# 0xPolygonZero/proof-protocol-decoder

Measured on AMD Instinct MI355X. Metric: txn-proofs/sec (whole node), 256-txn synthetic block, higher is better.
Workload: dtype u64 (Goldilocks field)

## Files before the change

### include/bpg.h

```cpp
#ifndef BPG_H
#define BPG_H
#include <stddef.h>
#include <stdint.h>

#ifdef __cplusplus
extern "C" {
#endif

typedef enum {
  BP_OK = 0,
  BP_ERR_ABORTED = -1,
  BP_ERR_INVALID_INPUT = -2,
  BP_ERR_RANGE = -3,
  BP_ERR_DEVICE = -4,
  BP_ERR_VERIFY = -5,
  BP_ERR_UNSUPPORTED = -6
} bp_status;

const char* bp_last_error(void);
const char* bp_version(void);
int bp_device_count(void);
int bp_use_blocking_sync(int device);
int bp_host_wait_mode(int device);



#define BP_NTT_MAX_COLS 65535u

enum { BP_NTT_FWD_BR2NAT = 0, BP_NTT_INV_NAT2BR = 1, BP_NTT_FWD_NAT = 2, BP_NTT_INV_NAT = 3 };
int bp_ntt_batch(uint64_t* d_cols, uint32_t log_n, uint32_t n_cols, uint64_t col_stride, int dir,
                 void* stream);

int bp_intt_batch(const uint64_t* d_values, uint64_t in_stride, uint64_t* d_coeffs_out, uint64_t out_stride,
                  uint32_t log_n, uint32_t n_cols, void* stream);

int bp_lde_batch(const uint64_t* d_in, uint64_t in_stride, uint64_t* d_coeffs_out, uint64_t coeffs_stride,
                 uint64_t* d_lde_out, uint64_t lde_stride, uint32_t log_n, uint32_t rate_bits,
                 uint32_t n_cols, int from_coeffs, void* stream);

int bp_debug_copy_u64(const uint64_t* d_in, uint64_t* d_out, uint64_t n, void* stream);

int bp_debug_field_ops(const uint64_t* d_a, const uint64_t* d_b, uint64_t* d_out, uint64_t n, void* stream);
int bp_debug_lazy_forms(const uint64_t* d_a, const uint64_t* d_b, uint64_t* d_out, uint64_t n, void* stream);
int bp_debug_mul_pow2(const uint64_t* d_a, uint64_t* d_out, uint64_t n, void* stream);

void bp_tune_quad_threshold(uint64_t n_perms);
void bp_tune_merkle_fused(int mode);
void bp_tune_merkle_wide(int log2_parents);
void bp_tune_poseidon_mx(int on);
void bp_tune_poseidon_mx_sets(int sets);
void bp_tune_poseidon_grouped(int on);
void bp_tune_assume_loaded(int mode);
void bp_tune_rec_batch(int n);
void bp_tune_side_lanes(int n);
void bp_tune_rec_riders(int on);
void bp_tune_txn_group(int n);
void bp_tune_rec_group(int mode);
int bp_debug_rec_batch_histogram(uint64_t* out, uint32_t n, int reset);
void bp_tune_witness_threads(int n);
void bp_tune_host_wait(int mode);
void bp_tune_host_poseidon(int mode);
int bp_debug_poseidon_host(uint64_t* states, size_t n);
void bp_tune_k5_spread(int on);
uint32_t bp_debug_poseidon_group_ops(uint32_t K);
int bp_debug_poseidon_group_tables(uint32_t K, uint32_t r0, uint8_t* out_ops, int32_t* out_cform, int32_t* out_cmain,
                                   int32_t* out_max_plane_sum);

void bp_tune_ntt_split(int mode);
void bp_tune_ntt_mx(int mode);
void bp_tune_reset(void);
int bp_debug_tune_state(char* buf, size_t cap);
int bp_debug_ntt_mx_tables(int kind, int inverse, uint8_t* out_a, int32_t* out_c, uint64_t* out_tw256,
                           uint64_t* out_tw16);
int bp_debug_poseidon_mx_cin(uint32_t* out);

int bp_poseidon_perm_batch(uint64_t* d_states, uint64_t n, void* stream);

uint64_t bp_merkle_digest_words(uint32_t log_leaves, uint32_t cap_height);
int bp_merkle_commit(const uint64_t* d_lde, uint64_t lde_stride, uint32_t n_cols, uint32_t log_n,
                     uint32_t rate_bits, uint32_t cap_height, uint64_t* d_digests, void* stream);

struct bp_stark_cfg;
typedef struct bp_air_family {
  uint32_t first_index, count;
  uint32_t kind;
  uint32_t degree;
} bp_air_family;
typedef struct bp_air_desc {
  uint32_t air_id;
  char name[24];
  uint32_t fixed_n_cols;
  uint32_t n_const_max;
  uint32_t degree;
  uint32_t n_cols, n_aux;
  uint32_t n_air_constraints, n_ctl_constraints;
  uint32_t n_units;
  uint32_t n_families;
  bp_air_family families[24];
} bp_air_desc;
uint32_t bp_air_count(void);
int bp_air_describe(uint32_t air_id, uint32_t n_cols, uint32_t n_const, uint32_t deg_pow, bp_air_desc* out);

int bp_air_register(const uint64_t* program, size_t n_words, uint32_t* air_id_out);
int bp_air_unregister(uint32_t air_id);
int bp_air_program_digest(uint32_t air_id, uint8_t out[32]);

uint64_t bp_quotient_scratch_words(uint32_t air_id, const struct bp_stark_cfg* shape);
int bp_quotient_eval(uint32_t air_id, const struct bp_stark_cfg* shape, const uint64_t* d_trace_lde,
                     const uint64_t* d_aux_lde, const uint64_t* d_const_lde, const uint64_t ctl[4],
                     const uint64_t alphas[2], uint64_t* d_scratch, uint64_t* d_qvals_out, void* stream);

int bp_air_port_products(uint32_t air_id, const struct bp_stark_cfg* shape, const uint64_t* d_trace, uint64_t stride,
                         const uint64_t* d_consts, const uint64_t pub[4], const uint64_t ctl[4], uint64_t* d_aux_out, void* stream);

int bp_range_multiplicities(const uint64_t* d_values, uint64_t stride, uint32_t n_cols, uint64_t n_rows, const uint64_t* d_filter,
                            uint32_t log_range, uint64_t* d_mult, uint64_t* first_bad, void* stream);
void bp_tune_range_lds_log(int log_range);

int bp_debug_air_aux(uint32_t air_id, const struct bp_stark_cfg* shape, const uint64_t* d_trace, const uint64_t ctl[4],
                     uint64_t* d_aux_out, void* stream);

typedef struct bp_air_violation {
  uint32_t row, constraint, family, kind;
  uint64_t value;
} bp_air_violation;
int bp_air_check_trace(uint32_t air_id, const struct bp_stark_cfg* shape, const uint64_t* d_trace, uint64_t stride,
                       const uint64_t* d_consts, const uint64_t pub[4], uint32_t max_rows, uint64_t* n_violated_rows,
// ... 274 lines not shown
```

### proof_protocol_decoder_amd/_abi.py

```python
import ctypes as C
from ctypes import POINTER as P

vp, cp, i, sz, dbl = C.c_void_p, C.c_char_p, C.c_int, C.c_size_t, C.c_double
u8, u32, u64, i32, i64 = C.c_uint8, C.c_uint32, C.c_uint64, C.c_int32, C.c_int64
u8p, u32p, u64p, i32p, szp = P(u8), P(u32), P(u64), P(i32), P(sz)
u8pp = P(u8p)

BP_OK, BP_ERR_ABORTED, BP_ERR_INVALID_INPUT, BP_ERR_RANGE, BP_ERR_DEVICE, BP_ERR_VERIFY, BP_ERR_UNSUPPORTED = 0, -1, -2, -3, -4, -5, -6
STATUS_NAMES = {v: k for k, v in list(globals().items()) if k == "BP_OK" or k.startswith("BP_ERR_")}
BP_SET_SKIP_LINK_CHECK = 1
BP_NUM_TABLES, BP_IR_WORDS, BP_PV_WORDS = 7, 25, 13

KNOBS = ("quad_threshold", "assume_loaded", "merkle_fused", "merkle_wide", "poseidon_mx", "poseidon_mx_sets",
         "poseidon_grouped", "ntt_mx", "ntt_split", "k5_spread", "host_wait", "host_poseidon", "rec_batch",
         "witness_threads", "side_lanes")


def _u32s(*names):
    return [(n, u32) for n in names]


class AirFamily(C.Structure):
    _fields_ = _u32s("first_index", "count", "kind", "degree")

# ... 94 lines not shown
    _fields_ = [("txn_number", u64), ("gas_used", u64), ("state_root", u64 * 4)]


class ShardOptions(C.Structure):
    _fields_ = _u32s("n_threads", "tree_shape")


ShardLeafFn = C.CFUNCTYPE(i, vp, u32, u8pp, szp)
ShardAggFn = C.CFUNCTYPE(i, vp, u8p, sz, i, u8p, sz, i, u8pp, szp)

_cfg, _conf, _wit, _opt, _gi = P(StarkCfg), P(BpConfig), P(TxnWitness), P(ShardOptions), P(GiOptions)
_trace = (i, [vp, u64, u32, vp, vp])
_check = [u32, _cfg, vp, u64, vp, u64p, u32, u64p, u32p, P(AirViolation), u32, u32p]
_knob, _ir_flag, _buf = (None, [i]), (i, [u64p, i]), [u8pp, szp]
PROTOTYPES = {
    "bp_last_error": (cp, []),
    "bp_version": (cp, []),
    "bp_device_count": (i, []),
    "bp_use_blocking_sync": (i, [i]),
    "bp_host_wait_mode": (i, [i]),
    "bp_ntt_batch": (i, [vp, u32, u32, u64, i, vp]),
    "bp_intt_batch": (i, [vp, u64, vp, u64, u32, u32, vp]),
    "bp_lde_batch": (i, [vp, u64, vp, u64, vp, u64, u32, u32, u32, i, vp]),
    "bp_debug_copy_u64": (i, [vp, vp, u64, vp]),
    "bp_debug_field_ops": (i, [vp, vp, vp, u64, vp]),
    "bp_debug_lazy_forms": (i, [vp, vp, vp, u64, vp]),
    "bp_debug_mul_pow2": (i, [vp, vp, u64, vp]),
    "bp_tune_quad_threshold": (None, [u64]),
    "bp_tune_merkle_fused": _knob,
    "bp_tune_merkle_wide": _knob,
    "bp_tune_poseidon_mx": _knob,
    "bp_tune_poseidon_mx_sets": _knob,
    "bp_tune_poseidon_grouped": _knob,
    "bp_tune_assume_loaded": _knob,
    "bp_tune_rec_batch": _knob,
    "bp_tune_side_lanes": _knob,
    "bp_tune_rec_riders": _knob,
    "bp_tune_txn_group": _knob,
    "bp_tune_rec_group": _knob,
    "bp_debug_rec_batch_histogram": (i, [u64p, u32, i]),
    "bp_tune_witness_threads": _knob,
    "bp_tune_host_wait": _knob,
    "bp_tune_host_poseidon": _knob,
    "bp_debug_poseidon_host": (i, [vp, sz]),
    "bp_tune_k5_spread": _knob,
    "bp_debug_poseidon_group_ops": (u32, [u32]),
    "bp_debug_poseidon_group_tables": (i, [u32, u32, u8p, i32p, i32p, i32p]),
    "bp_tune_ntt_split": _knob,
    "bp_tune_ntt_mx": _knob,
    "bp_tune_reset": (None, []),
    "bp_debug_tune_state": (i, [cp, sz]),
    "bp_debug_ntt_mx_tables": (i, [i, i, u8p, i32p, u64p, u64p]),
    "bp_debug_poseidon_mx_cin": (i, [u32p]),
    "bp_poseidon_perm_batch": (i, [vp, u64, vp]),
    "bp_merkle_digest_words": (u64, [u32, u32]),
    "bp_merkle_commit": (i, [vp, u64, u32, u32, u32, u32, vp, vp]),
    "bp_air_count": (u32, []),
    "bp_air_describe": (i, [u32, u32, u32, u32, P(AirDesc)]),
    "bp_air_register": (i, [vp, sz, u32p]),
    "bp_air_unregister": (i, [u32]),
    "bp_air_program_digest": (i, [u32, cp]),
    "bp_quotient_scratch_words": (u64, [u32, _cfg]),
    "bp_quotient_eval": (i, [u32, _cfg, vp, vp, vp, u64p, u64p, vp, vp, vp]),
    "bp_air_port_products": (i, [u32, _cfg, vp, u64, vp, u64p, u64p, vp, vp]),
    "bp_range_multiplicities": (i, [vp, u64, u32, u64, vp, u32, vp, u64p, vp]),
    "bp_tune_range_lds_log": _knob,
    "bp_debug_air_aux": (i, [u32, _cfg, vp, u64p, vp, vp]),
    "bp_air_check_trace": (i, _check + [vp]),
    "bp_air_check_trace_host": (i, _check),
    "bp_keccak_trace": _trace,
    "bp_logic_trace": _trace,
    "bp_memory_trace": _trace,
    "bp_arithmetic_trace": _trace,
    "bp_byte_packing_trace": _trace,
    "bp_keccak_sponge_trace": _trace,
    "bp_arithmetic_mul_trace": _trace,
    "bp_arithmetic_div_trace": (i, [vp, u32, vp, vp]),
    "bp_arithmetic_div_layout": (i, [u32p, sz]),
    "bp_arithmetic_mod_trace": (i, [vp, u32, vp, vp]),
    "bp_arithmetic_mod_layout": (i, [u32p, sz]),
    "bp_arithmetic_shift_trace": (i, [vp, u32, vp, vp]),
    "bp_arithmetic_shift_layout": (i, [u32p, sz]),
    "bp_arithmetic_sdiv_trace": (i, [vp, u32, vp, vp]),
    "bp_arithmetic_sdiv_layout": (i, [u32p, sz]),
    "bp_arithmetic_exp_trace": (i, [vp, u32, vp, u32, vp, vp]),
    "bp_arithmetic_exp_layout": (i, [u32p, sz]),
    "bp_plonk_constants": (i, [u64, u32, P(PlonkLayout), vp, vp]),
    "bp_plonk_trace": (i, [vp, u64, u64p, P(PlonkLayout), u64p, u32, vp, vp]),
    "bp_fri_fold": (i, [vp, u32, u32, u32, u64, u64p, vp, vp]),
    "bp_openings": (i, [vp, u64, u32, u32, u64p, u64p, vp, vp, vp]),
    "bp_pow_grind": (i, [u64p, u32, u32, u64p, vp]),
    "bp_stark_prove_synthetic": (i, [_cfg, u64, u64, i] + _buf),
    "bp_stark_prove_air": (i, [u32, _cfg, u64, u64, i] + _buf),
    "bp_stark_prove_trace": (i, [u32, _cfg, vp, u64, vp, u64p, i] + _buf),
    "bp_stark_verify_air": (i, [u32, _cfg, u64p, cp, sz]),
    "bp_stark_public_inputs": (None, [u64, u64p]),
    "bp_stark_public_input_list": (None, [u64, u64p]),
    "bp_stark_verify_air_pub": (i, [u32, _cfg, u64p, u64p, cp, sz]),
    "bp_stark_prove_table_set": (i, [P(SetTable), u32, P(SetLink), u32, u32, i] + _buf),
    "bp_stark_verify_table_set": (i, [P(SetTable), u32, P(u64p), P(SetLink), u32, cp, sz]),
    "bp_check_table_set": (i, [P(SetTable), u32, P(SetLink), u32, i, P(SetReport)]),
    "bp_release_cached_memory": (None, []),
    "bp_free_buffer": (None, [u8p]),
    "bp_config_default": (None, [_conf]),
    "bp_state_build": (i, [_conf, P(vp)]),
    "bp_state_free": (None, [vp]),
# ... 54 lines not shown
```

### proof_protocol_decoder_amd/csrc/air.hpp

```cpp
#pragma once
#include <cstdint>
#include <type_traits>
#include "gl.hpp"
#if defined(__HIP__)
#include "poseidon.cuh"
#endif

namespace bpg {
namespace air {

constexpr uint32_t SYNTHETIC = 0, KECCAK_F = 1, LOGIC = 2, MEMORY = 3, ARITHMETIC = 4, BYTE_PACKING = 5, KECCAK_SPONGE = 6, ARITHMETIC_MUL = 7, PLONK = 8, COUNT = 9;

struct Shape {
  uint32_t air_id, n_cols, n_const, deg_pow;
};

template <class T>
struct Ops;

#if defined(__HIP__)
template <>
struct Ops<uint64_t> {
  typedef uint64_t T;
  static __device__ __forceinline__ T k(uint64_t c) { return c; }
  static __device__ __forceinline__ T add(T a, T b) { return gl::addc(a, b); }
  static __device__ __forceinline__ T sub(T a, T b) { return gl::subc(a, b); }
  static __device__ __forceinline__ T mul(T a, T b) { return gl::mulc(a, b); }
  static __device__ __forceinline__ T dbl(T a) { return gl::addc(a, a); }
  static __device__ __forceinline__ void mul4(const T (&a)[4], const T (&b)[4], T (&r)[4]) {
    __builtin_amdgcn_sched_barrier(0);
    gl::mul_n<4>(a, b, r);
    gl::canon_n<4>(r);
    __builtin_amdgcn_sched_barrier(0);
  }
  static __device__ __forceinline__ void mul4_lazy(const T (&a)[4], const T (&b)[4], T (&r)[4]) {
    __builtin_amdgcn_sched_barrier(0);
    gl::mul_n<4>(a, b, r);
    __builtin_amdgcn_sched_barrier(0);
  }
  static __device__ __forceinline__ T add_lazy(T a_any, T b) { return gl::add(a_any, b); }
  static __device__ __forceinline__ T sub_lazy(T a_any, T b) { return gl::sub(a_any, b); }
  static __device__ __forceinline__ T mul7(T a_any) { return gl::mul7(a_any); }
};
#endif
template <>
struct Ops<gl::Ext> {
  typedef gl::Ext T;
  static T k(uint64_t c) { return gl::ext(c); }
  static T add(T a, T b) { return gl::add(a, b); }
  static T sub(T a, T b) { return gl::sub(a, b); }
  static T mul(T a, T b) { return gl::mul(a, b); }
  static T dbl(T a) { return gl::add(a, a); }
  static void mul4(const T (&a)[4], const T (&b)[4], T (&r)[4]) {
    for (int i = 0; i < 4; i++) r[i] = gl::mul(a[i], b[i]);
  }
  static void mul4_lazy(const T (&a)[4], const T (&b)[4], T (&r)[4]) { mul4(a, b, r); }
  static T add_lazy(T a, T b) { return gl::add(a, b); }
  static T sub_lazy(T a, T b) { return gl::sub(a, b); }
  static T mul7(T a) { return gl::scale(a, 7); }
};

GL_HD uint64_t poseidon_rc(uint32_t i) {
  constexpr uint64_t RC[360] = {
#include "poseidon_rc.inc"
  };
  return RC[i];
}
GL_HD uint32_t poseidon_mds_entry(uint32_t r, uint32_t c) {
  constexpr uint32_t C[12] = {17, 15, 41, 16, 2, 28, 13, 13, 39, 18, 34, 20};
  return C[(c + 12 - r) % 12] + ((r | c) == 0 ? 8u : 0u);
}
template <class T>
struct PoseidonOps {
  typedef Ops<T> F;
  static GL_HD T sbox(T x) {
    const T x2 = F::mul(x, x), x4 = F::mul(x2, x2), x3 = F::mul(x2, x);
    return F::mul(x3, x4);
  }
  static GL_HD void sbox_all(T (&s)[12]) {
    for (uint32_t i = 0; i < 12; i++) s[i] = sbox(s[i]);
  }
  static GL_HD void mds_rc(T (&s)[12], int next) {
    T o[12];
    for (uint32_t r = 0; r < 12; r++) {
      T acc = F::k(next >= 0 ? poseidon_rc(12 * (uint32_t)next + r) : 0);
      for (uint32_t c = 0; c < 12; c++) acc = F::add(acc, F::mul(F::k(poseidon_mds_entry(r, c)), s[c]));
      o[r] = acc;
    }
    for (uint32_t r = 0; r < 12; r++) s[r] = o[r];
  }
  static GL_HD void mds_rc_word0(T (&s)[12], int next) { mds_rc(s, next); }
  static GL_HD T add_rc0(T x, uint32_t i) { return F::add(x, F::k(poseidon_rc(i))); }
};
#if defined(__HIP__)
template <>
struct PoseidonOps<uint64_t> {
  static __device__ __forceinline__ uint64_t sbox(uint64_t x) { return gl::canon(poseidon::sbox(x)); }
  static __device__ __forceinline__ void sbox_all(uint64_t (&s)[12]) { poseidon::sbox_all(s); }
  static __device__ __forceinline__ void mds_rc(uint64_t (&s)[12], int next) {
    if (next >= 0) poseidon::mds<true>(s, poseidon::RC + 12 * next);
    else poseidon::mds<false>(s, nullptr);
#pragma unroll
    for (int i = 0; i < 12; i++) s[i] = gl::canon(s[i]);
  }
  static __device__ __forceinline__ void mds_rc_word0(uint64_t (&s)[12], int next) {
    poseidon::mds<true>(s, poseidon::RC + 12 * next);
    s[0] = gl::canon(s[0]);
  }
  static __device__ __forceinline__ uint64_t add_rc0(uint64_t x, uint32_t i) { return gl::addc(x, poseidon::RC[i]); }
};
#endif

namespace synthetic {
GL_HD uint32_t n_constraints(const Shape& s) { return 3 * (s.n_cols / 4); }
GL_HD uint32_t per_unit(const Shape& s) {
  const uint32_t G = s.n_cols / 4, u = (G + 47) / 48;
  return u < 8 ? 8 : u;
}
GL_HD uint32_t n_units(const Shape& s) {
  const uint32_t G = s.n_cols / 4, pu = per_unit(s);
  return (G + pu - 1) / pu;
}
template <class T, class Row, class Emit>
GL_HD void eval_unit(const Shape& s, uint32_t unit, const Row& row, Emit& out) {
  typedef Ops<T> F;
  const uint32_t G = s.n_cols / 4, pu = per_unit(s), g0 = unit * pu, g1 = g0 + pu < G ? g0 + pu : G;
#pragma unroll 1
  for (uint32_t g = g0; g < g1; g++) {
    const T a = row.loc(4 * g), b = row.loc(4 * g + 1), c = row.loc(4 * g + 2), d = row.loc(4 * g + 3);
    const T dn = row.nxt(4 * g + 3);
    const T q = s.n_const ? row.cst(g % s.n_const) : F::k(1);
    const T x4[4] = {a, q, a, a}, y4[4] = {b, a, b, b};
    T p4[4];
    F::mul4(x4, y4, p4);
    const T ab = p4[0], qa = p4[1];
    T t = F::mul(ab, c);
    if (s.deg_pow == 3) t = F::mul(F::mul(t, t), t);
    out.all(3 * g, F::sub(F::sub(c, ab), qa));
    out.transition(3 * g + 1, F::sub(F::sub(dn, t), b));
    out.first(3 * g + 2, F::sub(F::sub(d, a), b));
  }
}
}

namespace keccak {
constexpr uint32_t N_COLS = 2431, N_CONSTRAINTS = 2826, N_UNITS = 11;
constexpr uint32_t COL_STEP = 0, COL_A = 24, COL_C = 74, COL_CP = 394, COL_AP = 714, COL_APP = 2314, COL_APP0_BITS = 2364,
                   COL_APPP = 2428, COL_G = 2430;
constexpr uint32_t F0 = 0, F1 = 24, F2 = 48, F3 = 2032, F4 = 2352, F5 = 2672, F6 = 2722, F7 = 2772, F8 = 2774, F9 = 2776;
GL_HD uint64_t round_constant(uint32_t i) {
  constexpr uint64_t RC[24] = {
      0x0000000000000001ULL, 0x0000000000008082ULL, 0x800000000000808aULL, 0x8000000080008000ULL,
      0x000000000000808bULL, 0x0000000080000001ULL, 0x8000000080008081ULL, 0x8000000000008009ULL,
      0x000000000000008aULL, 0x0000000000000088ULL, 0x0000000080008009ULL, 0x000000008000000aULL,
      0x000000008000808bULL, 0x800000000000008bULL, 0x8000000000008089ULL, 0x8000000000008003ULL,
      0x8000000000008002ULL, 0x8000000000000080ULL, 0x000000000000800aULL, 0x800000008000000aULL,
      0x8000000080008081ULL, 0x8000000000008080ULL, 0x0000000080000001ULL, 0x8000000080008008ULL};
  return RC[i];
}
GL_HD uint32_t rho(uint32_t l) {
  constexpr uint8_t R[25] = {0, 1, 62, 28, 27, 36, 44, 6, 55, 20, 3, 10, 43, 25, 39, 41, 45, 15, 21, 8, 18, 2, 61, 56, 14};
  return R[l];
// ... 607 lines not shown
        const uint32_t j = col - H_OUT;
        if (l + 1 == L.depth) { const uint32_t i = L.path_pi0 + 8 * p + 4 + j; col_out = i & 7; row_out = HASH_ROW0 + (i >> 3); }
        else { col_out = H_IN + j; row_out = row + 1; }
      }
    } else if (L.leaf_len && row >= leaf_row0(L) && row < leaf_row0(L) + leaf_rows(L)) {
      const uint32_t LH = hash_rows(L.leaf_len), t = row - leaf_row0(L), p = t / LH, h = t % LH;
      if (col < 12) {
        if (hash_word_is_carried(L.leaf_len, h, col)) {
          if (h > 0) { col_out = H_OUT + col; row_out = row - 1; }
          else if (col < 11) col_out = col + 1;
          else if (p + 1 < L.n_paths) { col_out = 8; row_out = row + LH; }
          else { col_out = MERKLE_ZERO_COL; row_out = ZERO_ROW; }
        }
      } else if (col < 24) {
        const uint32_t k = col - H_OUT;
        if (h + 1 == LH) {
          if (k < 4) { const uint32_t i = L.path_pi0 + 8 * p + k; col_out = i & 7; row_out = HASH_ROW0 + (i >> 3); }
        } else if (hash_word_is_carried(L.leaf_len, h + 1, k)) {
          col_out = H_IN + k; row_out = row + 1;
        }
      }
    }
    return;
  }
  const uint32_t g = row >> 2, p = row & 3, s = col >> 2, w = col & 3;
  const uint32_t base = 4 * g;
  if (p == 0) {
    if (w == 3) { col_out = 4 * s; row_out = base + 1; }
    else if (w == 2) { col_out = col; row_out = base + 1; }
  } else if (p == 1) {
    if (w == 0) { col_out = 4 * ((s + N_SLOTS - 1) % N_SLOTS) + 1; row_out = base + 1; }
    else if (w == 1) { col_out = 4 * ((s + 1) % N_SLOTS) + 3; row_out = base; }
    else if (w == 2) {
      if (base == A0 && s < 4) { col_out = H_OUT + s; row_out = last_hash_row; }
      else { col_out = col; row_out = base; }
    } else if (s < N_SBOX) { col_out = 4 * s; row_out = base + 2; }
  } else if (p == 2) {
    if (s < N_SBOX && w == 0) { col_out = 4 * s + 3; row_out = base + 1; }
    else if (s < N_SBOX && w == 3) { col_out = 4 * s; row_out = base + 3; }
  } else {
    if (s < N_SBOX && w == 0) { col_out = 4 * s + 3; row_out = base + 2; }
  }
}
GL_HD uint64_t chunk_shift(uint32_t u) {
  constexpr uint64_t K8[10] = {0x1ULL, 0x57f6c1ULL, 0x1e39a5057d81ULL, 0x62b942f056949437ULL, 0x33cdc3006affab59ULL,
                               0xcb893e19494e73dULL, 0x36f01f6fb02d9400ULL, 0xd844c68aea81b372ULL, 0x9c232dfb69ab851eULL,
                               0x255bd1d3b936892aULL};
  return K8[u];
}
template <class T, class Row, class Emit, bool SELECTOR = true>
GL_HD void eval_hash_unit(const Row& row, Emit& out) {
  typedef Ops<T> F;
  typedef PoseidonOps<T> H;
  const T qh = row.cst(CST_HASH);
  const T q4[4] = {qh, qh, qh, qh};
  T st[12];
  {
    const T sw = row.loc(H_SWAP);
    T lhs[4], rhs[4], dl[4], pr[4], g[4];
#pragma unroll
    for (uint32_t i = 0; i < 4; i++) {
      lhs[i] = row.loc(H_IN + i);
      rhs[i] = row.loc(H_IN + 4 + i);
      dl[i] = row.loc(H_DELTA + i);
      pr[i] = F::sub(rhs[i], lhs[i]);
    }
    const T s4[4] = {sw, sw, sw, sw};
    F::mul4(s4, pr, g);
#pragma unroll
    for (uint32_t i = 0; i < 4; i++) {
      const T d = F::sub(dl[i], g[i]);
      out.all(G5 + 1 + i, SELECTOR ? F::mul(qh, d) : d);
      st[i] = H::add_rc0(F::add(lhs[i], dl[i]), i);
      st[4 + i] = H::add_rc0(F::sub(rhs[i], dl[i]), 4 + i);
      st[8 + i] = H::add_rc0(row.loc(H_IN + 8 + i), 8 + i);
    }
    const T bit = F::mul(sw, F::sub(sw, F::k(1)));
    out.all(G5, SELECTOR ? F::mul(qh, bit) : bit);
  }
  auto check12 = [&](uint32_t col0, uint32_t idx0) {
#pragma unroll
    for (uint32_t i0 = 0; i0 < 12; i0 += 4) {
      T d[4], g[4];
#pragma unroll
      for (uint32_t i = 0; i < 4; i++) {
        const T wv = row.loc(col0 + i0 + i);
        d[i] = F::sub(wv, st[i0 + i]);
        st[i0 + i] = wv;
      }
      if (SELECTOR) F::mul4(q4, d, g);
#pragma unroll
      for (uint32_t i = 0; i < 4; i++) out.all(idx0 + i0 + i, SELECTOR ? g[i] : d[i]);
    }
  };
#pragma unroll 1
  for (uint32_t r = 1; r <= 3; r++) {
    H::sbox_all(st);
    H::mds_rc(st, (int)r);
    check12(H_FULL1 + 12 * (r - 1), G4 + 12 * (r - 1));
  }
  H::sbox_all(st);
  H::mds_rc_word0(st, 4);
#pragma unroll 1
  for (uint32_t r = 4; r <= 25; r++) {
    const T pv = row.loc(H_PART + r - 4);
    const T d = F::sub(pv, st[0]);
    out.all(G4 + 36 + (r - 4), SELECTOR ? F::mul(qh, d) : d);
    st[0] = H::sbox(pv);
    if (r < 25) H::mds_rc_word0(st, (int)r + 1);
    else H::mds_rc(st, (int)r + 1);
  }
#pragma unroll 1
  for (uint32_t r = 26; r <= 29; r++) {
    check12(H_FULL2 + 12 * (r - 26), G4 + 58 + 12 * (r - 26));
    H::sbox_all(st);
    H::mds_rc(st, r < 29 ? (int)r + 1 : -1);
  }
  check12(H_OUT, G4 + 106);
}
template <class T, class Row, class Emit>
GL_HD void eval_chunk_unit(uint32_t u, uint32_t ctl_base, const uint64_t ctl[4], const Row& row, Emit& out) {
  typedef Ops<T> F;
  T w[8], sg[8];
#pragma unroll
  for (uint32_t i = 0; i < 8; i++) w[i] = row.loc(8 * u + i);
#pragma unroll
  for (uint32_t i = 0; i < 8; i++) sg[i] = row.cst(CST_SIGMA + 8 * u + i);
  const T qa = row.cst(CST_ARITH), qs = row.cst(CST_SBOX), c0 = row.cst(CST_C0), c1 = row.cst(CST_C1);
  const T x = row.x(), kp = F::k(chunk_shift(u));
  const T beta[2] = {F::k(ctl[0]), F::k(ctl[2])}, gamma[2] = {F::k(ctl[1]), F::k(ctl[3])};
  T bkx[2];
  {
    const T l1[4] = {w[0], w[4], c1, c1}, r1[4] = {w[1], w[5], w[2], w[6]};
    T p1[4];
    F::mul4(l1, r1, p1);
    const T l2[4] = {c0, c0, beta[0], beta[1]}, r2[4] = {p1[0], p1[1], x, x};
    T p2[4];
    F::mul4(l2, r2, p2);
    const T t0 = F::sub(F::add(p2[0], p1[2]), w[3]), t1 = F::sub(F::add(p2[1], p1[3]), w[7]);
    const T l3[4] = {qa, qa, p2[2], p2[3]}, r3[4] = {t0, t1, kp, kp};
    T p3[4];
    F::mul4(l3, r3, p3);
    out.all(G0 + 2 * u, p3[0]);
    out.all(G0 + 2 * u + 1, p3[1]);
    bkx[0] = p3[2];
    bkx[1] = p3[3];
  }
  T half[2][4];
#pragma unroll
  for (uint32_t c = 0; c < 2; c++) {
    const T b4[4] = {beta[c], beta[c], beta[c], beta[c]};
    T pn[4], pd[4];
#pragma unroll
    for (uint32_t h = 0; h < 2; h++) {
      const T s4[4] = {sg[4 * h], sg[4 * h + 1], sg[4 * h + 2], sg[4 * h + 3]};
      T bs[4], tn[4], td[4];
      F::mul4_lazy(b4, s4, bs);
#pragma unroll
      for (uint32_t i = 0; i < 4; i++) {
        const T wg = F::add(w[4 * h + i], gamma[c]);
        tn[i] = F::add_lazy(bkx[c], wg);
        td[i] = F::add_lazy(bs[i], wg);
        bkx[c] = F::mul7(bkx[c]);
      }
// ... 371 lines not shown
```

### proof_protocol_decoder_amd/csrc/air_check.hip

```cpp
#include <algorithm>
#include "air_check.hpp"
#include "common.hpp"
#include "gl.hpp"
#include "air.hpp"
#include "air_check_dev.cuh"
#include "air_program.hpp"

namespace {

using bpg::CheckArgs;
using namespace bpg::chk;

template <uint32_t AIR>
__global__ void __launch_bounds__(256) air_check_kernel(CheckArgs a) {
  const uint64_t n = (uint64_t)1 << a.log_n;
  const uint64_t pos = blockIdx.x * (uint64_t)blockDim.x + threadIdx.x;
  uint64_t r0 = 0, r1 = 0;
  if (pos < n) {
    CheckEmit out = check_emit(a, pos);
    const CheckRow row = check_row(a, pos, AIR == bpg::air::PLONK);
    const bpg::air::Shape shape{AIR, a.n_cols, a.n_const, a.deg_pow};
    const uint64_t ctl[4] = {0, 0, 0, 0};
    const uint32_t u0 = blockIdx.y * a.units_per_wg, u1 = min(u0 + a.units_per_wg, a.n_units);
#pragma unroll 1
    for (uint32_t u = u0; u < u1; u++) {
      bpg::air::eval_unit_of<AIR, uint64_t>(shape, u, a.T, ctl, row, out);
    }
    r0 = out.result(0);
    r1 = out.result(1);
  }
  if (a.partial) {
    if (pos < n) {
      a.partial[((uint64_t)blockIdx.y * 2) * n + pos] = r0;
      a.partial[((uint64_t)blockIdx.y * 2 + 1) * n + pos] = r1;
    }
    return;
  }
  flag_rows(a, pos, (r0 | r1) != 0);
}
__global__ void __launch_bounds__(256) air_check_plonk_hash_kernel(CheckArgs a, uint32_t wg_row) {
  const uint64_t n = (uint64_t)1 << a.log_n;
  const uint64_t pos = blockIdx.x * (uint64_t)blockDim.x + threadIdx.x;
  if (pos >= n) return;
  CheckEmit out = check_emit(a, pos);
  const CheckRow row = check_row(a, pos, false);
  bpg::air::plonk::eval_hash_unit<uint64_t, CheckRow, CheckEmit, false>(row, out);
  const uint64_t qh = row.cst(bpg::air::plonk::CST_HASH);
  a.partial[((uint64_t)wg_row * 2) * n + pos] = gl::mulc(out.result(0), qh);
  a.partial[((uint64_t)wg_row * 2 + 1) * n + pos] = gl::mulc(out.result(1), qh);
}
__global__ void __launch_bounds__(256) air_check_reduce_kernel(CheckArgs a, uint32_t n_rows) {
  const uint64_t n = (uint64_t)1 << a.log_n;
  const uint64_t pos = blockIdx.x * (uint64_t)blockDim.x + threadIdx.x;
  uint64_t r0 = 0, r1 = 0;
  if (pos < n)
    for (uint32_t c = 0; c < n_rows; c++) {
      r0 = gl::addc(r0, a.partial[((uint64_t)c * 2) * n + pos]);
      r1 = gl::addc(r1, a.partial[((uint64_t)c * 2 + 1) * n + pos]);
    }
  flag_rows(a, pos, (r0 | r1) != 0);
}
__global__ void __launch_bounds__(256) air_check_alpha_kernel(uint64_t* apow, uint32_t T, uint64_t a0, uint64_t a1) {
  const uint32_t e = blockIdx.x * blockDim.x + threadIdx.x;
  if (e >= T) return;
  apow[(uint64_t)blockIdx.y * T + e] = gl::pow(blockIdx.y ? a1 : a0, e);
}
__global__ void __launch_bounds__(256) air_check_gather_kernel(const uint64_t* trace, uint64_t stride, uint32_t n_cols,
                                                               const uint32_t* rows, uint64_t* out) {
  const uint32_t c = blockIdx.x * blockDim.x + threadIdx.x;
  if (c >= n_cols) return;
  out[(uint64_t)blockIdx.y * n_cols + c] = trace[(uint64_t)c * stride + rows[blockIdx.y]];
}

}

namespace bpg {

uint64_t air_check_partial_words(CheckArgs& a) {
  const air::Shape shape{a.air_id, a.n_cols, a.n_const, a.deg_pow};
  const bool plonk = a.air_id == air::PLONK;
  a.n_units = plonk ? air::plonk::N_UNITS - 1 : air::any_n_units(shape);
  const uint64_t blocks = ceil_div((uint64_t)1 << a.log_n, 256);
  if (blocks >= 512 || a.n_units == 1) {
    a.units_per_wg = a.n_units;
  } else {
    const uint32_t want = (uint32_t)std::min<uint64_t>(a.n_units, ceil_div(1024, blocks));
    a.units_per_wg = ceil_div(a.n_units, want);
  }
  a.wg_rows = ceil_div(a.n_units, a.units_per_wg);
  const uint32_t rows = a.wg_rows + (plonk ? 1 : 0);
  return rows > 1 ? 2 * ((uint64_t)rows << a.log_n) : 0;
}

int launch_air_check(const CheckArgs& a, hipStream_t st) {
  const uint64_t n = (uint64_t)1 << a.log_n;
  BPG_HIP(hipMemsetAsync(a.count, 0, sizeof(unsigned long long), st));
  air_check_alpha_kernel<<<dim3(ceil_div(a.T, 256), 2), 256, 0, st>>>(const_cast<uint64_t*>(a.apow), a.T, a.alpha0, a.alpha1);
  BPG_LAUNCH_CHECK();
  const dim3 g1(ceil_div(n, 256), a.wg_rows);
  if (air::prog::is_registered(a.air_id)) {
    if (int rc = launch_air_check_program(a, g1, st)) return rc;
  } else air::dispatch(a.air_id, [&](auto A) { air_check_kernel<A.value><<<g1, 256, 0, st>>>(a); });
// ... 22 lines not shown
```

### proof_protocol_decoder_amd/csrc/stark_kernels.hip

```cpp
#include "common.hpp"
#include "gl.hpp"
#include "poseidon.cuh"
#include "poseidon_mx.cuh"
#include "stark_kernels.hpp"
#include "arg_ring.hpp"
#include "quotient_dev.cuh"
#include "air_program.hpp"

namespace {

using gl::Ext;
using namespace bpg::k5;

__device__ __forceinline__ uint64_t splitmix64(uint64_t x) {
  uint64_t z = x + 0x9E3779B97F4A7C15ULL;
  z = (z ^ (z >> 30)) * 0xBF58476D1CE4E5B9ULL;
  z = (z ^ (z >> 27)) * 0x94D049BB133111EBULL;
  return z ^ (z >> 31);
}
__device__ __forceinline__ uint64_t rnd(uint64_t seed, uint64_t col, uint64_t row) {
  return gl::canon(splitmix64(seed ^ (col << 32) ^ row));
}
__device__ __forceinline__ uint64_t pow_e(uint64_t t, uint32_t e) {
  return e == 3 ? gl::mulc(gl::mulc(t, t), t) : t;
// ... 707 lines not shown
__global__ void __launch_bounds__(256) __attribute__((amdgpu_waves_per_eu(AIR == bpg::air::KECCAK_F ? 3 : 1)))
quotient_air_kernel(bpg::ArgPtr<bpg::QuotArgs> args) {
  BPG_ARG_BATCH(bpg::QuotArgs, args);
  if (gridDim.x * gridDim.y * gridDim.z <= 64) __builtin_amdgcn_s_setprio(3);
  const bpg::QuotArgs& q = batch[blockIdx.z];
  const uint64_t rows = (uint64_t)1 << (q.log_n + q.rate_bits);
  const uint64_t pos = blockIdx.x * (uint64_t)blockDim.x + threadIdx.x;
  if (pos >= rows) return;
  const uint32_t n = 1u << q.log_n;
  const uint32_t t = (uint32_t)(pos >> q.log_n), m = (uint32_t)(pos & (n - 1));
  DevEmit out{q.apow, q.n_constraints, row_point(q, t, m),
              {gl::dot_zero(), gl::dot_zero(), gl::dot_zero(), gl::dot_zero()}, 0, 0, false};
  DevRow row{q.trace_lde, q.aux_lde, q.const_lde, q.trace_stride, q.aux_stride, q.const_stride, pos,
             ((uint64_t)t << q.log_n) | ((m + 1) & (n - 1)), out.rp.x, q.ctl.pub};
  const bpg::air::Shape shape{AIR, q.n_cols, q.n_const, q.deg_pow};
  const uint32_t n_units = q.n_air_units + q.n_ctl_units;
  const uint32_t u0 = blockIdx.y * q.units_per_wg, u1 = min(u0 + q.units_per_wg, n_units);
#pragma unroll 1
  for (uint32_t u = u0; u < u1; u++) {
    if (u < q.n_air_units) {
      bpg::air::eval_unit_of<AIR, uint64_t>(shape, u, q.n_air_constraints, q.ctl.v, row, out);
    } else {
      const uint32_t k0 = (u - q.n_air_units) * q.aux_per_unit, k1 = min(k0 + q.aux_per_unit, q.n_aux);
      const bpg::air::Shape cs{AIR, q.n_cols, q.n_const, q.deg_pow};
      bpg::air::ctl::eval<uint64_t>(cs, q.n_air_constraints, k0, k1, q.ctl.v, row, out);
    }
  }
  const uint64_t r0 = out.result(0), r1 = out.result(1);
  if (gridDim.y == 1 && q.side_rows == 0) {
    const uint64_t zh_inv = q.apow[2 * (size_t)q.n_constraints + 32 + t];
    q.qvals[pos] = gl::mulc(r0, zh_inv);
    q.qvals[rows + pos] = gl::mulc(r1, zh_inv);
  } else {
    q.partial[((uint64_t)blockIdx.y * 2) * rows + pos] = r0;
    q.partial[((uint64_t)blockIdx.y * 2 + 1) * rows + pos] = r1;
  }
}
__global__ void __launch_bounds__(256) __attribute__((amdgpu_waves_per_eu(BPG_PLONK_HASH_WAVES)))
quotient_plonk_hash_kernel(bpg::ArgPtr<bpg::QuotArgs> args, uint32_t wg_row) {
  BPG_ARG_BATCH(bpg::QuotArgs, args);
  if (gridDim.x * gridDim.y * gridDim.z <= 64) __builtin_amdgcn_s_setprio(3);
  const bpg::QuotArgs& q = batch[blockIdx.z];
  const uint64_t rows = (uint64_t)1 << (q.log_n + q.rate_bits);
  const uint64_t pos = blockIdx.x * (uint64_t)blockDim.x + threadIdx.x;
  if (pos >= rows) return;
  const uint32_t n = 1u << q.log_n;
  const uint32_t t = (uint32_t)(pos >> q.log_n), m = (uint32_t)(pos & (n - 1));
  DevEmit out{q.apow, q.n_constraints, row_point(q, t, m),
              {gl::dot_zero(), gl::dot_zero(), gl::dot_zero(), gl::dot_zero()}, 0, 0, false};
  DevRow row{q.trace_lde, q.aux_lde, q.const_lde, q.trace_stride, q.aux_stride, q.const_stride, pos,
             ((uint64_t)t << q.log_n) | ((m + 1) & (n - 1)), out.rp.x, q.ctl.pub};
  bpg::air::plonk::eval_hash_unit<uint64_t, DevRow, DevEmit, false>(row, out);
  const uint64_t qh = row.cst(bpg::air::plonk::CST_HASH);
  q.partial[((uint64_t)wg_row * 2) * rows + pos] = gl::mulc(out.result(0), qh);
  q.partial[((uint64_t)wg_row * 2 + 1) * rows + pos] = gl::mulc(out.result(1), qh);
}
__global__ void __launch_bounds__(256) quotient_sum_kernel(bpg::ArgPtr<bpg::QuotArgs> args, uint32_t n_wg_rows) {
  BPG_ARG_BATCH(bpg::QuotArgs, args);
  if (gridDim.x * gridDim.y * gridDim.z <= 64) __builtin_amdgcn_s_setprio(3);
  const bpg::QuotArgs& q = batch[blockIdx.z];
  const uint64_t rows = (uint64_t)1 << (q.log_n + q.rate_bits);
  const uint64_t pos = blockIdx.x * (uint64_t)blockDim.x + threadIdx.x;
  if (pos >= rows) return;
  const uint32_t j = blockIdx.y, t = (uint32_t)(pos >> q.log_n);
  uint64_t acc = 0;
  for (uint32_t c = 0; c < n_wg_rows; c++) acc = gl::addc(acc, q.partial[((uint64_t)c * 2 + j) * rows + pos]);
  q.qvals[(uint64_t)j * rows + pos] = gl::mulc(acc, q.apow[2 * (size_t)q.n_constraints + 32 + t]);
}
struct CosetTab {
  uint64_t v[48];
};
struct AlphaTabArgs {
  uint64_t* out;
  uint64_t a0, a1;
};
__global__ void __launch_bounds__(256)
alpha_table_kernel(bpg::ArgPtr<AlphaTabArgs> args, uint32_t T, CosetTab ct) {
  BPG_ARG_BATCH(AlphaTabArgs, args);
  if (gridDim.x * gridDim.y * gridDim.z <= 64) __builtin_amdgcn_s_setprio(3);
  uint64_t* __restrict__ out = batch[blockIdx.z].out;
  const uint64_t a0 = batch[blockIdx.z].a0, a1 = batch[blockIdx.z].a1;
  const uint32_t e = blockIdx.x * blockDim.x + threadIdx.x;
  if (blockIdx.y == 0 && e < 48) out[2 * (uint64_t)T + e] = ct.v[e];
  if (e >= T) return;
  out[(uint64_t)blockIdx.y * T + e] = gl::pow(blockIdx.y ? a1 : a0, e);
}
__global__ void __launch_bounds__(256) quotient_chunks_kernel(bpg::ArgPtr<bpg::ChunkArgs> args) {
  BPG_ARG_BATCH(bpg::ChunkArgs, args);
  if (gridDim.x * gridDim.y * gridDim.z <= 64) __builtin_amdgcn_s_setprio(3);
  const bpg::ChunkArgs& c = batch[blockIdx.z];
  const uint32_t pos = blockIdx.x * blockDim.x + threadIdx.x, n = 1u << c.log_n;
  if (pos >= n) return;
  const uint32_t j = blockIdx.y, R = 1u << c.rate_bits;
  const uint64_t* e = c.e + (uint64_t)j * ((uint64_t)n << c.rate_bits);
  uint64_t d[16];
  for (uint32_t t = 0; t < R; t++) d[t] = gl::mulc(e[(uint64_t)t * n + pos], c.inv_scale[(uint64_t)t * n + pos]);
  for (uint32_t n1 = 0; n1 < R; n1++) {
    uint64_t acc = 0;
    for (uint32_t t = 0; t < R; t++) acc = gl::addc(acc, gl::mulc(d[t], c.wr_inv_pow[(t * n1) & (R - 1)]));
    c.out[((uint64_t)j * R + n1) * c.out_stride + pos] = gl::mulc(acc, c.chunk_scale[n1]);
  }
}

__global__ void __launch_bounds__(256)
power_vector_kernel(bpg::ArgPtr<bpg::PowerVecArgs> args, uint32_t log_n) {
  BPG_ARG_BATCH(bpg::PowerVecArgs, args);
  if (gridDim.x * gridDim.y * gridDim.z <= 64) __builtin_amdgcn_s_setprio(3);
  const uint32_t pos = blockIdx.x * blockDim.x + threadIdx.x, n = 1u << log_n;
// ... 761 lines not shown
    else if (ns == 2) fri_layer_leaf_mx_kernel<2><<<dim3(ceil_div(n, 128), 1, batch), 256, 0, st>>>(ab);
    else fri_layer_leaf_mx_kernel<1><<<dim3(ceil_div(n, 64), 1, batch), 256, 0, st>>>(ab);
  } else if (n * batch < quad_threshold()) fri_layer_leaf_quad_kernel<<<dim3(ceil_div(n * 4, 256), 1, batch), 256, 0, st>>>(ab);
  else fri_layer_leaf_kernel<<<dim3(ceil_div(n, 256), 1, batch), 256, 0, st>>>(ab);
  BPG_LAUNCH_CHECK();
  return BP_OK;
}
int launch_fri_fold(const FriLayerArgs* a, uint32_t batch, hipStream_t st) {
  if (int rc = check_batch(batch)) return rc;
  uint64_t n = (uint64_t)1 << (a[0].log_nl - a[0].arity_bits + a[0].rate_bits);
  BPG_ARG_BLOCKS(ab, a, batch, st);
  KernelTimer kt(PROF_FRI_FOLD, st, 16.0 * (double)n * ((1 << a[0].arity_bits) + 1) * batch, true);
  BPG_LAUNCH_TIMED(kt, fri_fold_kernel, dim3(ceil_div(n, 256), 1, batch), 256, 0, st, ab);
  BPG_LAUNCH_CHECK();
  return BP_OK;
}
int launch_pow(const PowArgs* a, uint32_t batch, uint32_t n_candidates, unsigned long long* d_result, hipStream_t st) {
  if (int rc = check_batch(batch)) return rc;
  BPG_ARG_BLOCKS(ab, a, batch, st);
  const dim3 grid(n_candidates / 256, 1, batch);
  if (poseidon_mx()) {
    const uint32_t* gtab = group_tables();
    if (gtab) pow_grind_mx_kernel<true><<<grid, 256, 0, st>>>(ab, d_result, gtab);
    else pow_grind_mx_kernel<false><<<grid, 256, 0, st>>>(ab, d_result, nullptr);
  } else
    pow_grind_kernel<<<grid, 256, 0, st>>>(ab, d_result);
  BPG_LAUNCH_CHECK();
  return BP_OK;
}
int launch_query_initial(const QueryArgs& a, uint32_t batch, uint32_t n_oracles, hipStream_t st) {
  if (int rc = check_batch(batch)) return rc;
  if (!a.n_queries || a.n_queries * batch > MAX_BATCH_QUERIES) return fail(BP_ERR_INVALID_INPUT, "query launch: %u x %u indices, at most %u", a.n_queries, batch, MAX_BATCH_QUERIES);
  dim3 grid(a.n_queries * batch, n_oracles);
  const QueryArgs* ab = nullptr;
  if (int rc = arg_put(st, &a, 1, &ab)) return rc;
  query_initial_kernel<<<grid, 256, 0, st>>>(arg_ptr(ab));
  BPG_LAUNCH_CHECK();
  return BP_OK;
}
int launch_query_layers(const QueryLayerArgs& a, uint32_t batch, uint32_t n_layers, hipStream_t st) {
  if (!n_layers) return BP_OK;
  if (int rc = check_batch(batch)) return rc;
  if (!a.n_queries || a.n_queries * batch > MAX_BATCH_QUERIES || n_layers > MAX_FRI_LAYERS)
    return fail(BP_ERR_INVALID_INPUT, "query launch: %u x %u indices, %u layers", a.n_queries, batch, n_layers);
  dim3 grid(a.n_queries * batch, n_layers);
  const QueryLayerArgs* ab = nullptr;
  if (int rc = arg_put(st, &a, 1, &ab)) return rc;
  query_layers_kernel<<<grid, 64, 0, st>>>(arg_ptr(ab));
  BPG_LAUNCH_CHECK();
  return BP_OK;
}

}
```

Baseline: 38.73.

## Fold three Poseidon partial rounds into precomputed linear forms in the plonk hash gate

Replaces the per-round partial-round loop in the plonk hash constraint evaluation on device with groups of three rounds. Each group is computed as constexpr-precomputed composed MDS linear forms with folded round constants, accumulated in split 32-bit lanes and reduced once per group. It also drops per-round canonicalisation by negating the constraint differences (NEG_DIFF) and compensating with a negation at the partial-sum store. This cuts the modular reductions and MDS work in the quotient hash kernel, at the cost of larger coefficient tables, more register pressure and a correctness dependence on the accumulator bound static_assert.

Result: no change. 39.04 (median of 6 runs) (+0.8%).

```diff
diff --git a/include/bpg.h b/include/bpg.h
--- a/include/bpg.h
+++ b/include/bpg.h
@@ -73,6 +73,7 @@
 int bp_debug_ntt_mx_tables(int kind, int inverse, uint8_t* out_a, int32_t* out_c, uint64_t* out_tw256,
                            uint64_t* out_tw16);
 int bp_debug_poseidon_mx_cin(uint32_t* out);
+int bp_debug_poseidon_partial_forms(uint32_t* out_coef, uint64_t* out_const, uint64_t* out_bound);
 
 int bp_poseidon_perm_batch(uint64_t* d_states, uint64_t n, void* stream);
 
diff --git a/proof_protocol_decoder_amd/_abi.py b/proof_protocol_decoder_amd/_abi.py
--- a/proof_protocol_decoder_amd/_abi.py
+++ b/proof_protocol_decoder_amd/_abi.py
@@ -170,6 +170,7 @@
     "bp_debug_tune_state": (i, [cp, sz]),
     "bp_debug_ntt_mx_tables": (i, [i, i, u8p, i32p, u64p, u64p]),
     "bp_debug_poseidon_mx_cin": (i, [u32p]),
+    "bp_debug_poseidon_partial_forms": (i, [u32p, u64p, u64p]),
     "bp_poseidon_perm_batch": (i, [vp, u64, vp]),
     "bp_merkle_digest_words": (u64, [u32, u32]),
     "bp_merkle_commit": (i, [vp, u64, u32, u32, u32, u32, vp, vp]),
diff --git a/proof_protocol_decoder_amd/csrc/air.hpp b/proof_protocol_decoder_amd/csrc/air.hpp
--- a/proof_protocol_decoder_amd/csrc/air.hpp
+++ b/proof_protocol_decoder_amd/csrc/air.hpp
@@ -70,9 +70,93 @@
   constexpr uint32_t C[12] = {17, 15, 41, 16, 2, 28, 13, 13, 39, 18, 34, 20};
   return C[(c + 12 - r) % 12] + ((r | c) == 0 ? 8u : 0u);
 }
+namespace pforms {
+constexpr uint32_t GROUPS = 7, ROUNDS = 3, FIRST = 4, N_COEF = 12 + 12 + 1 + 144 + 12 + 12, N_CONST = 14;
+constexpr uint64_t ACC_BOUND = (uint64_t)1 << 56;
+struct Tables {
+  uint32_t a1[12];
+  uint32_t a2[12];
+  uint32_t b2;
+  uint32_t a3[12][12];
+  uint32_t b3[12];
+  uint32_t c3[12];
+  uint64_t k[GROUPS][N_CONST];
+  uint64_t worst_sum;
+};
+constexpr uint64_t PRIME = 0xFFFFFFFF00000001ULL;
+constexpr uint64_t addm(uint64_t a, uint64_t b) {
+  const uint64_t s = a + b;
+  return (s < a || s >= PRIME) ? s - PRIME : s;
+}
+constexpr uint64_t mulm_small(uint64_t a, uint32_t c) {
+  const uint64_t lo = (a & 0xFFFFFFFFu) * c, t = (a >> 32) * c;
+  const uint64_t t_hi = t >> 32, t_lo = t & 0xFFFFFFFFu;
+  const uint64_t mid = t_lo << 32;
+  return addm(addm(lo, mid >= PRIME ? mid - PRIME : mid), t_hi * 0xFFFFFFFFu);
+}
+constexpr Tables make_partial_forms() {
+  constexpr uint64_t rc[360] = {
+#include "poseidon_rc.inc"
+  };
+  constexpr uint32_t circ[12] = {17, 15, 41, 16, 2, 28, 13, 13, 39, 18, 34, 20};
+  Tables t{};
+  uint64_t M[12][12] = {}, EM[12][12] = {}, MEM[12][12] = {}, EMEM[12][12] = {}, MEMEM[12][12] = {};
+  for (uint32_t r = 0; r < 12; r++)
+    for (uint32_t c = 0; c < 12; c++) {
+      M[r][c] = circ[(c + 12 - r) % 12] + ((r | c) == 0 ? 8u : 0u);
+      EM[r][c] = r ? M[r][c] : 0;
+    }
+  for (uint32_t r = 0; r < 12; r++)
+    for (uint32_t c = 0; c < 12; c++)
+      for (uint32_t j = 0; j < 12; j++) MEM[r][c] += M[r][j] * EM[j][c];
+  for (uint32_t r = 0; r < 12; r++)
+    for (uint32_t c = 0; c < 12; c++) EMEM[r][c] = r ? MEM[r][c] : 0;
+  for (uint32_t r = 0; r < 12; r++)
+    for (uint32_t c = 0; c < 12; c++)
+      for (uint32_t j = 0; j < 12; j++) MEMEM[r][c] += M[r][j] * EMEM[j][c];
+  uint64_t s1 = 0, s2 = M[0][0], worst = 0;
+  for (uint32_t c = 0; c < 12; c++) {
+    t.a1[c] = (uint32_t)M[0][c];
+    t.a2[c] = (uint32_t)MEM[0][c];
+    s1 += M[0][c];
+    s2 += MEM[0][c];
+  }
+  t.b2 = (uint32_t)M[0][0];
+  worst = s1 > s2 ? s1 : s2;
+  for (uint32_t r = 0; r < 12; r++) {
+    uint64_t s3 = MEM[r][0] + M[r][0];
+    for (uint32_t c = 0; c < 12; c++) {
+      t.a3[r][c] = (uint32_t)MEMEM[r][c];
+      s3 += MEMEM[r][c];
+    }
+    t.b3[r] = (uint32_t)MEM[r][0];
+    t.c3[r] = (uint32_t)M[r][0];
+    worst = s3 > worst ? s3 : worst;
+  }
+  t.worst_sum = worst;
+  for (uint32_t g = 0; g < GROUPS; g++) {
+    const uint64_t *c1 = rc + 12 * (FIRST + ROUNDS * g + 1), *c2 = c1 + 12, *c3 = c2 + 12;
+    t.k[g][0] = c1[0];
+    uint64_t k2 = c2[0];
+    for (uint32_t j = 1; j < 12; j++) k2 = addm(k2, mulm_small(c1[j], (uint32_t)M[0][j]));
+    t.k[g][1] = k2;
+    for (uint32_t r = 0; r < 12; r++) {
+      uint64_t k3 = c3[r];
+      for (uint32_t j = 1; j < 12; j++)
+        k3 = addm(addm(k3, mulm_small(c2[j], (uint32_t)M[r][j])), mulm_small(c1[j], (uint32_t)MEM[r][j]));
+      t.k[g][2 + r] = k3;
+    }
+  }
+  return t;
+}
+static_assert(make_partial_forms().worst_sum * 0xFFFFFFFFull + ((uint64_t)1 << 32) < ACC_BOUND,
+              "a three-round accumulator of the gate's partial rounds outgrows mxa::reduce_rows");
+}
+
 template <class T>
 struct PoseidonOps {
   typedef Ops<T> F;
+  static constexpr bool NEG_DIFF = false;
   static GL_HD T sbox(T x) {
     const T x2 = F::mul(x, x), x4 = F::mul(x2, x2), x3 = F::mul(x2, x);
     return F::mul(x3, x4);
@@ -91,23 +175,114 @@
   }
   static GL_HD void mds_rc_word0(T (&s)[12], int next) { mds_rc(s, next); }
   static GL_HD T add_rc0(T x, uint32_t i) { return F::add(x, F::k(poseidon_rc(i))); }
+  template <class Wire, class Check>
+  static GL_HD void partial_rounds(T (&s)[12], const Wire& wire, const Check& check) {
+    mds_rc_word0(s, 4);
+#pragma unroll 1
+    for (uint32_t r = 4; r <= 25; r++) {
+      const T pv = wire(r - 4);
+      check(r - 4, s[0], pv);
+      s[0] = sbox(pv);
+      if (r < 25) mds_rc_word0(s, (int)r + 1);
+      else mds_rc(s, (int)r + 1);
+    }
+  }
 };
 #if defined(__HIP__)
+static __constant__ pforms::Tables PARTIAL_FORMS = pforms::make_partial_forms();
 template <>
 struct PoseidonOps<uint64_t> {
-  static __device__ __forceinline__ uint64_t sbox(uint64_t x) { return gl::canon(poseidon::sbox(x)); }
+  static constexpr bool NEG_DIFF = true;
   static __device__ __forceinline__ void sbox_all(uint64_t (&s)[12]) { poseidon::sbox_all(s); }
   static __device__ __forceinline__ void mds_rc(uint64_t (&s)[12], int next) {
     if (next >= 0) poseidon::mds<true>(s, poseidon::RC + 12 * next);
     else poseidon::mds<false>(s, nullptr);
-#pragma unroll
-    for (int i = 0; i < 12; i++) s[i] = gl::canon(s[i]);
-  }
-  static __device__ __forceinline__ void mds_rc_word0(uint64_t (&s)[12], int next) {
-    poseidon::mds<true>(s, poseidon::RC + 12 * next);
-    s[0] = gl::canon(s[0]);
   }
   static __device__ __forceinline__ uint64_t add_rc0(uint64_t x, uint32_t i) { return gl::addc(x, poseidon::RC[i]); }
+  template <class Wire, class Check>
+  static __device__ __forceinline__ void partial_rounds(uint64_t (&s)[12], const Wire& wire, const Check& check) {
+    constexpr pforms::Tables t = pforms::make_partial_forms();
+    poseidon::mds<true>(s, poseidon::RC + 12 * 4);
+    {
+      const uint64_t w = wire(0);
+      check(0, s[0], w);
+      s[0] = poseidon::sbox(w);
+    }
+#pragma unroll 1
+    for (uint32_t g = 0; g < pforms::GROUPS; g++) {
+      const uint64_t* __restrict__ k = PARTIAL_FORMS.k[g];
+      uint32_t z = 0;
+      asm volatile("" : "+s"(z));
+      auto lit = [&](uint32_t cf) { return cf > 64 ? cf + z : cf; };
+      const uint64_t w[3] = {wire(3 * g + 1), wire(3 * g + 2), wire(3 * g + 3)};
+      uint64_t sg[3] = {w[0], w[1], w[2]};
+      poseidon::sbox_n<3>(sg);
+      __builtin_amdgcn_sched_barrier(0);
+      uint32_t lo[14], hi[14];
+#pragma unroll
+      for (int i = 0; i < 12; i++) {
+        lo[i] = (uint32_t)s[i];
+        hi[i] = (uint32_t)(s[i] >> 32);
+      }
+#pragma unroll
+      for (int i = 0; i < 2; i++) {
+        lo[12 + i] = (uint32_t)sg[i];
+        hi[12 + i] = (uint32_t)(sg[i] >> 32);
+      }
+      auto acc = [&](int v, uint64_t& L, uint64_t& H) {
+        const uint64_t kv = k[v];
+        const int r = v >= 2 ? v - 2 : 0;
+        L = (uint32_t)kv;
+        H = kv >> 32;
+#pragma unroll
+        for (int c = 0; c < 12; c++) {
+          const uint32_t cf = lit(v == 0 ? t.a1[c] : v == 1 ? t.a2[c] : t.a3[r][c]);
+          L += (uint64_t)lo[c] * cf;
+          H += (uint64_t)hi[c] * cf;
+        }
+        if (v >= 1) {
+          const uint32_t cf = lit(v == 1 ? t.b2 : t.b3[r]);
+          L += (uint64_t)lo[12] * cf;
+          H += (uint64_t)hi[12] * cf;
+        }
+        if (v >= 2) {
+          const uint32_t cf = lit(t.c3[r]);
+          L += (uint64_t)lo[13] * cf;
+          H += (uint64_t)hi[13] * cf;
+        }
+      };
+      uint64_t chk[2];
+      {
+        uint64_t L[4], H[4], o[4];
+#pragma unroll
+        for (int i = 0; i < 4; i++) acc(i, L[i], H[i]);
+        mxa::reduce_rows<4>(L, H, o);
+        chk[0] = o[0]; chk[1] = o[1]; s[0] = o[2]; s[1] = o[3];
+      }
+      {
+        uint64_t L[4], H[4], o[4];
+#pragma unroll
+        for (int i = 0; i < 4; i++) acc(4 + i, L[i], H[i]);
+        mxa::reduce_rows<4>(L, H, o);
+#pragma unroll
+        for (int i = 0; i < 4; i++) s[2 + i] = o[i];
+      }
+#pragma unroll
+      for (int q = 0; q < 2; q++) {
+        uint64_t L[3], H[3], o[3];
+#pragma unroll
+        for (int i = 0; i < 3; i++) acc(8 + 3 * q + i, L[i], H[i]);
+        mxa::reduce_rows<3>(L, H, o);
+#pragma unroll
+        for (int i = 0; i < 3; i++) s[6 + 3 * q + i] = o[i];
+      }
+      check(3 * g + 1, chk[0], w[0]);
+      check(3 * g + 2, chk[1], w[1]);
+      check(3 * g + 3, s[0], w[2]);
+      s[0] = sg[2];
+    }
+    poseidon::mds<true>(s, poseidon::RC + 12 * 26);
+  }
 };
 #endif
 
@@ -821,8 +996,9 @@
 GL_HD void eval_hash_unit(const Row& row, Emit& out) {
   typedef Ops<T> F;
   typedef PoseidonOps<T> H;
-  const T qh = row.cst(CST_HASH);
-  const T q4[4] = {qh, qh, qh, qh};
+  auto diff = [](T wire, T state) { return H::NEG_DIFF ? F::sub_lazy(state, wire) : F::sub(wire, state); };
+  const T qh = row.cst(CST_HASH), qn = H::NEG_DIFF ? F::sub(F::k(0), qh) : qh;
+  const T q4[4] = {qn, qn, qn, qn};
   T st[12];
   {
     const T sw = row.loc(H_SWAP);
@@ -838,13 +1014,13 @@
     F::mul4(s4, pr, g);
 #pragma unroll
     for (uint32_t i = 0; i < 4; i++) {
-      const T d = F::sub(dl[i], g[i]);
-      out.all(G5 + 1 + i, SELECTOR ? F::mul(qh, d) : d);
+      const T d = diff(dl[i], g[i]);
+      out.all(G5 + 1 + i, SELECTOR ? F::mul(qn, d) : d);
       st[i] = H::add_rc0(F::add(lhs[i], dl[i]), i);
       st[4 + i] = H::add_rc0(F::sub(rhs[i], dl[i]), 4 + i);
       st[8 + i] = H::add_rc0(row.loc(H_IN + 8 + i), 8 + i);
     }
-    const T bit = F::mul(sw, F::sub(sw, F::k(1)));
+    const T bit = F::mul(sw, H::NEG_DIFF && !SELECTOR ? F::sub(F::k(1), sw) : F::sub(sw, F::k(1)));
     out.all(G5, SELECTOR ? F::mul(qh, bit) : bit);
   }
   auto check12 = [&](uint32_t col0, uint32_t idx0) {
@@ -854,7 +1030,7 @@
 #pragma unroll
       for (uint32_t i = 0; i < 4; i++) {
         const T wv = row.loc(col0 + i0 + i);
-        d[i] = F::sub(wv, st[i0 + i]);
+        d[i] = diff(wv, st[i0 + i]);
         st[i0 + i] = wv;
       }
       if (SELECTOR) F::mul4(q4, d, g);
@@ -869,16 +1045,12 @@
     check12(H_FULL1 + 12 * (r - 1), G4 + 12 * (r - 1));
   }
   H::sbox_all(st);
-  H::mds_rc_word0(st, 4);
-#pragma unroll 1
-  for (uint32_t r = 4; r <= 25; r++) {
-    const T pv = row.loc(H_PART + r - 4);
-    const T d = F::sub(pv, st[0]);
-    out.all(G4 + 36 + (r - 4), SELECTOR ? F::mul(qh, d) : d);
-    st[0] = H::sbox(pv);
-    if (r < 25) H::mds_rc_word0(st, (int)r + 1);
-    else H::mds_rc(st, (int)r + 1);
-  }
+  H::partial_rounds(
+      st, [&](uint32_t k) { return row.loc(H_PART + k); },
+      [&](uint32_t k, T state0, T wire) {
+        const T d = diff(wire, state0);
+        out.all(G4 + 36 + k, SELECTOR ? F::mul(qn, d) : d);
+      });
 #pragma unroll 1
   for (uint32_t r = 26; r <= 29; r++) {
     check12(H_FULL2 + 12 * (r - 26), G4 + 58 + 12 * (r - 26));
diff --git a/proof_protocol_decoder_amd/csrc/air_check.hip b/proof_protocol_decoder_amd/csrc/air_check.hip
--- a/proof_protocol_decoder_amd/csrc/air_check.hip
+++ b/proof_protocol_decoder_amd/csrc/air_check.hip
@@ -46,8 +46,8 @@
   const CheckRow row = check_row(a, pos, false);
   bpg::air::plonk::eval_hash_unit<uint64_t, CheckRow, CheckEmit, false>(row, out);
   const uint64_t qh = row.cst(bpg::air::plonk::CST_HASH);
-  a.partial[((uint64_t)wg_row * 2) * n + pos] = gl::mulc(out.result(0), qh);
-  a.partial[((uint64_t)wg_row * 2 + 1) * n + pos] = gl::mulc(out.result(1), qh);
+  a.partial[((uint64_t)wg_row * 2) * n + pos] = gl::mulc(gl::negc(out.result(0)), qh);
+  a.partial[((uint64_t)wg_row * 2 + 1) * n + pos] = gl::mulc(gl::negc(out.result(1)), qh);
 }
 __global__ void __launch_bounds__(256) air_check_reduce_kernel(CheckArgs a, uint32_t n_rows) {
   const uint64_t n = (uint64_t)1 << a.log_n;
diff --git a/proof_protocol_decoder_amd/csrc/stark_kernels.hip b/proof_protocol_decoder_amd/csrc/stark_kernels.hip
--- a/proof_protocol_decoder_amd/csrc/stark_kernels.hip
+++ b/proof_protocol_decoder_amd/csrc/stark_kernels.hip
@@ -783,8 +783,8 @@
              ((uint64_t)t << q.log_n) | ((m + 1) & (n - 1)), out.rp.x, q.ctl.pub};
   bpg::air::plonk::eval_hash_unit<uint64_t, DevRow, DevEmit, false>(row, out);
   const uint64_t qh = row.cst(bpg::air::plonk::CST_HASH);
-  q.partial[((uint64_t)wg_row * 2) * rows + pos] = gl::mulc(out.result(0), qh);
-  q.partial[((uint64_t)wg_row * 2 + 1) * rows + pos] = gl::mulc(out.result(1), qh);
+  q.partial[((uint64_t)wg_row * 2) * rows + pos] = gl::mulc(gl::negc(out.result(0)), qh);
+  q.partial[((uint64_t)wg_row * 2 + 1) * rows + pos] = gl::mulc(gl::negc(out.result(1)), qh);
 }
 __global__ void __launch_bounds__(256) quotient_sum_kernel(bpg::ArgPtr<bpg::QuotArgs> args, uint32_t n_wg_rows) {
   BPG_ARG_BATCH(bpg::QuotArgs, args);
@@ -1652,3 +1652,23 @@
 }
 
 }
+
+extern "C" int bp_debug_poseidon_partial_forms(uint32_t* out_coef, uint64_t* out_const, uint64_t* out_bound) {
+  namespace pf = bpg::air::pforms;
+  if (!out_coef || !out_const || !out_bound) return bpg::fail(BP_ERR_INVALID_INPUT, "bp_debug_poseidon_partial_forms: null buffer");
+  static const pf::Tables t = pf::make_partial_forms();
+  uint32_t* o = out_coef;
+  for (int c = 0; c < 12; c++) *o++ = t.a1[c];
+  for (int c = 0; c < 12; c++) *o++ = t.a2[c];
+  *o++ = t.b2;
+  for (int r = 0; r < 12; r++)
+    for (int c = 0; c < 12; c++) *o++ = t.a3[r][c];
+  for (int r = 0; r < 12; r++) *o++ = t.b3[r];
+  for (int r = 0; r < 12; r++) *o++ = t.c3[r];
+  static_assert(pf::N_COEF == 193, "the layout include/bpg.h states");
+  for (uint32_t g = 0; g < pf::GROUPS; g++)
+    for (uint32_t j = 0; j < pf::N_CONST; j++) out_const[g * pf::N_CONST + j] = t.k[g][j];
+  out_bound[0] = t.worst_sum;
+  out_bound[1] = pf::ACC_BOUND;
+  return BP_OK;
+}
```
